# KelestZ/Latent2im

Measured on AMD Instinct MI355X. Metric: edited images/sec, higher is better.
Workload: dtype f32; 1 GPU; StyleGAN2 FFHQ-shaped 1024^2 generator (random-init, noise weights ~ 0.05: per-layer noise drawn every pass), ResNet-50 regressor, 1 CelebA attr (train.py flow), full loss (reg+content+GAN), batch 8 per GPU, linear W+ walk, eager launches; resolution=1024, global_batch=8, per_gpu_batch=8, losses=reg+content+gan, parallelism=dp1, loss_branch_streams=3, hip_graph=False

## Files before the change

include/l2i.h:

```cpp
#ifndef L2I_H
#define L2I_H

#include <stdint.h>

#ifdef __cplusplus
extern "C" {
#endif

#define L2I_OK 0
#define L2I_E_ARG (-1)
#define L2I_E_LAUNCH (-2)
#define L2I_E_UNSUPPORTED (-3)

#define L2I_ACT_NONE 0
#define L2I_ACT_LRELU 1
#define L2I_ACT_RELU 2

typedef struct l2i_conv_params {
    const float* x;
    const float* w;
    float* y;
    int32_t B, Cin, H, W, Cout, CoutP;
    int32_t KH, KW, stride, pad_y, pad_x;
    int32_t OH, OW, OHf, OWf;
// ... 19 lines not shown
    const float* res_sub;
    float res_coef;
    const float* res_coef_dev;
    const float* sq_ref;
    float* sq_out;
    int64_t w_bstride;
    int32_t out_f32;
    int32_t in_h8;
    const float* rgb_w;
    const float* rgb_bias;
    float* rgb_out;
    float* pool_out;
    uint8_t* pool_idx;
    uint8_t* mask_out;
    int32_t mask_bits;
} l2i_conv_params;
#define L2I_SQ_SLOTS 1024

int l2i_conv2d_f32(const l2i_conv_params* p, void* stream);

#define L2I_FAMILY_IMPLICIT_GEMM 0
#define L2I_FAMILY_GEMM1X1 1
#define L2I_FAMILY_CIN3 2
#define L2I_FAMILY_DIRECT_SMALL 3
int l2i_conv2d_family(const l2i_conv_params* p);

int l2i_conv_transpose2d_f32(const l2i_conv_params* p, void* stream);

int l2i_conv2d_bf16x3_f32(const l2i_conv_params* p, void* stream);

int l2i_conv_transpose2d_bf16x3_f32(const l2i_conv_params* p, void* stream);

int l2i_conv2d_wino_f32(const l2i_conv_params* p, void* stream);

int l2i_conv2d_wino4_f32(const l2i_conv_params* p, void* stream);
#define L2I_WINO4S_LEAN_CLASSES 8
int l2i_wino4s_epilogue_class(const l2i_conv_params* p);

int l2i_conv2d_h8(const l2i_conv_params* p, void* stream);
int l2i_conv_transpose2d_h8(const l2i_conv_params* p, void* stream);
// ... 169 lines not shown
```

latent2im_amd/_lib.py:

```python
import ctypes
import os

import torch

_HERE = os.path.dirname(os.path.abspath(__file__))
LIB_PATH = os.environ.get('L2I_LIB') or os.path.join(_HERE, 'libl2i_hip.so')

ACT_NONE, ACT_LRELU, ACT_RELU = 0, 1, 2

c_f = ctypes.c_float
c_i = ctypes.c_int32
c_p = ctypes.c_void_p
c_l = ctypes.c_int64


class ConvParams(ctypes.Structure):
    _fields_ = [
        ('x', c_p), ('w', c_p), ('y', c_p),
        ('B', c_i), ('Cin', c_i), ('H', c_i), ('W', c_i), ('Cout', c_i), ('CoutP', c_i),
        ('KH', c_i), ('KW', c_i), ('stride', c_i), ('pad_y', c_i), ('pad_x', c_i),
        ('OH', c_i), ('OW', c_i), ('OHf', c_i), ('OWf', c_i),
        ('oy_step', c_i), ('ox_step', c_i), ('oy_off', c_i), ('ox_off', c_i),
        ('in_scale', c_p), ('in_mask', c_p), ('mask_pos', c_f), ('mask_neg', c_f),
        ('out_scale', c_p), ('noise', c_p), ('noise_w', c_f), ('bias', c_p),
        ('residual', c_p), ('res_mask', c_p), ('out_mask', c_p),
        ('act', c_i), ('act_slope', c_f), ('act_gain', c_f), ('out_gain', c_f),
        ('accumulate', c_i), ('tile_hint', c_i),
        ('w_hi', c_p), ('w_lo', c_p),
        ('ws', c_p), ('ksplit', c_i), ('res_sub', c_p), ('res_coef', c_f), ('res_coef_dev', c_p),
        ('sq_ref', c_p), ('sq_out', c_p),
        ('w_bstride', c_l), ('out_f32', c_i),
        ('in_h8', c_i), ('rgb_w', c_p), ('rgb_bias', c_p), ('rgb_out', c_p), ('pool_out', c_p), ('pool_idx', c_p),
        ('mask_out', c_p), ('mask_bits', c_i),
    ]


SQ_SLOTS = 1024
WINO4S_LEAN_CLASSES = 8


class SegmvPart(ctypes.Structure):
    _fields_ = [('K', c_i), ('in_off_c', c_i), ('in_off_b', c_i), ('in_bstride', c_i), ('w_pitch', c_i), ('pre', c_i), ('aux_off', c_i), ('pad_', c_i),
                ('w_off', c_l)]


class SegmvSeg(ctypes.Structure):
    _fields_ = [('rows', c_i), ('nparts', c_i), ('out_off_c', c_i), ('out_off_b', c_i), ('out_bstride', c_i), ('epi', c_i), ('bias_off', c_i),
                ('e_off_c', c_i), ('e_off_b', c_i), ('e_bstride', c_i), ('rgb_off_b', c_i), ('rgb_w_off', c_i), ('part', SegmvPart * 2)]


_SIGNATURES = {
    'l2i_conv2d_f32': (c_i, [ctypes.POINTER(ConvParams), c_p]),
    'l2i_conv2d_family': (c_i, [ctypes.POINTER(ConvParams)]),
    'l2i_conv_transpose2d_f32': (c_i, [ctypes.POINTER(ConvParams), c_p]),
    'l2i_conv2d_bf16x3_f32': (c_i, [ctypes.POINTER(ConvParams), c_p]),
    'l2i_conv_transpose2d_bf16x3_f32': (c_i, [ctypes.POINTER(ConvParams), c_p]),
    'l2i_conv2d_wino_f32': (c_i, [ctypes.POINTER(ConvParams), c_p]),
    'l2i_conv2d_wino4_f32': (c_i, [ctypes.POINTER(ConvParams), c_p]),
    'l2i_wino4s_epilogue_class': (c_i, [ctypes.POINTER(ConvParams)]),
    'l2i_conv1x1_pair_f32': (c_i, [ctypes.POINTER(ConvParams), ctypes.POINTER(ConvParams), c_p]),
    'l2i_conv2d_h8': (c_i, [ctypes.POINTER(ConvParams), c_p]),
    'l2i_conv_transpose2d_h8': (c_i, [ctypes.POINTER(ConvParams), c_p]),
    'l2i_conv_img_h8': (c_i, [ctypes.POINTER(ConvParams), c_p]),
    'l2i_conv1x1_pair_h8': (c_i, [ctypes.POINTER(ConvParams), ctypes.POINTER(ConvParams), c_i, c_p]),
    'l2i_conv_chain3_h8': (c_i, [ctypes.POINTER(ConvParams), ctypes.POINTER(ConvParams), ctypes.POINTER(ConvParams), c_i, c_p]),
    'l2i_fused_bias_act_f32': (c_i, [c_p, c_p, c_p, c_p, c_l, c_l, c_l, c_i, c_i, c_f, c_f, c_p]),
    'l2i_fused_bias_act_f16': (c_i, [c_p, c_p, c_p, c_p, c_l, c_l, c_l, c_i, c_i, c_f, c_f, c_p]),
    'l2i_upfirdn2d_f16': (c_i, [c_p, c_p, c_p, c_l, c_i, c_i, c_i, c_i, c_i, c_i, c_i, c_i, c_i, c_i, c_i, c_i, c_p]),
# ... 154 lines not shown
```

latent2im_amd/conv.py:

```python

import numpy as np
import torch

from . import _lib
from ._lib import ACT_LRELU, ACT_NONE, ACT_RELU, ConvParams


import os as _os

PRECISION = _os.environ.get('L2I_PRECISION', 'f32')
H8_PRECISIONS = ('bf16', 'f16')


def h8_dtype():
    return torch.float16 if PRECISION == 'f16' else torch.bfloat16

USE_WINOGRAD = True
WINO4_MODES = ('all', 'tall', 'r4', 'off')
WINO4 = 'all'
WINO4_R4_MIN_W = 64
SPLIT_K = True
_WS = {}
USE_FUSED_TRANSPOSED = True
PROFILE = None
FAMILIES = ('implicit_gemm_f32', 'gemm1x1_f32', 'cin3_f32', 'direct_small_valu')
FAMILY_INFO = {
    'winograd_f32': ('conv_wino_kernel', 16.0 / 36.0, 157.3),
    'winograd4_f32': ('conv_wino4s_kernel', 36.0 / 144.0, 157.3),
    'implicit_gemm_f32': ('conv_mfma_kernel / conv3x3s2_dma_kernel', 1.0, 157.3),
    'gemm1x1_f32': ('gemm1x1_kernel', 1.0, 157.3),
    'transposed_f32': ('convt_mfma_kernel', 1.0, 157.3),
    'cin3_f32': ('conv_cin3_kernel', 28.0 / 27.0, 157.3),
    'direct_small_valu': ('conv_direct_small_kernel', 1.0, 157.3),
    'implicit_gemm_bf16x3': ('conv_bf16x3_pipe_kernel', 3.0, 2500.0),
    'transposed_bf16x3': ('conv_bf16x3_pipe_kernel<TR>', 3.0, 2500.0),
    'conv_h8': ('conv_h8_kernel', 1.0, 2500.0),
# ... 290 lines not shown
        B, cg, H, W, _ = x.shape
        cin = cg * 8
        assert x.dtype in (torch.bfloat16, torch.float16) and x.is_contiguous()
    else:
        B, cin, H, W = x.shape
    assert cin == F.cin and y.shape[0] == B and y.shape[1] == F.cout and y.dtype == torch.float32
    OHf, OWf = y.shape[2], y.shape[3]
    p = _conv_params(x, F.w, y, B, cin, H, W, F.cout, F.k, F.k, 2, F.pad, F.pad, (OHf + 1) // 2, (OWf + 1) // 2, OHf, OWf, 2, in_mask=in_mask, mask=mask,
                     out_gain=out_gain)
    p.in_h8 = 0 if not h8 else (2 if x.dtype == torch.float16 else 1)
    _launch('l2i_conv_transpose2d_f32', (p,), None, _transposed_meta, p, 'direct_small_valu')
    return y


def _split_k(p, px, cin, y):
    if not (SPLIT_K and px <= 2048 and cin >= 256):
        return
    ks = 16 if px <= 128 else (8 if px <= 512 else 4)
    while ks > 1 and (cin % ks or (cin // ks) % 2 or cin // ks < 16):
        ks //= 2
    if ks > 1:
        need = ks * y.numel()
        key = (y.device, torch.cuda.current_stream(y.device).cuda_stream)
        ws = _WS.get(key)
        if ws is None or ws.numel() < need:
            ws = _WS[key] = torch.empty(max(need, 1 << 22), device=y.device, dtype=torch.float32)
        p.ws, p.ksplit = _lib.fptr(ws), ks


def run_fused_transposed(F, x, y, in_scale=None, in_mask=None, mask=(1.0, 0.0), out_scale=None, out_gain=1.0, tile_hint=0):
    B, cin, H, W = x.shape
    assert cin == F.cin and y.shape[0] == B and y.shape[1] == F.cout
    OHf, OWf = y.shape[2], y.shape[3]
    p = _conv_params(x, F.w, y, B, cin, H, W, F.cout, F.k, F.k, 2, F.pad, F.pad, (OHf + 1) // 2, (OWf + 1) // 2, OHf, OWf, 2, in_scale=in_scale,
                     in_mask=in_mask, mask=mask, out_scale=out_scale, out_gain=out_gain)
    p.tile_hint = tile_hint
    name, family = 'l2i_conv_transpose2d_f32', 'transposed_f32'
    nat_h, nat_w = (H - 1) * 2 - 2 * F.pad + F.k, (W - 1) * 2 - 2 * F.pad + F.k
    if (PRECISION == 'bf16x3' and tile_hint == 0 and F.w_src is not None and W % 4 == 0 and W >= 32 and x.data_ptr() % 16 == 0
            and (in_mask is None or in_mask.data_ptr() % 16 == 0) and 0 <= OHf - nat_h <= 8 and 0 <= OWf - nat_w <= 8):
        planes = F.bf16x3_planes()
        p.w_hi, p.w_lo = _lib.ptr(planes[0]), _lib.ptr(planes[1])
# ... 356 lines not shown
```

latent2im_amd/csrc/l2i_conv.hip:

```cpp

#include <hip/hip_runtime.h>
#include <stdint.h>
#include <type_traits>
#include "l2i.h"
#include "l2i_internal.h"
#include "l2i_device.h"
#include "l2i_epilogue.h"


struct ConvLaunch {
    int tw_log2, th_log2, tb_log2;
    int tiles_x, tiles_y, bgroups, mblocks;
    int CK;
    int IH, IW, IWp;
    int planeS, plane;
    int rows_c;
    unsigned magic_iw, magic_rc, magic_ih;
    int in_elems;
    int w_vec;
    int vec_epi;
    int lstride, gstep;
    int total;
    int ksplit, cin_per;
};

template <int BM> struct WSlots { static constexpr int value = (BM == 128) ? 10 : (BM == 64 ? 8 : 4); };

template <int WM, int WN, bool VEC, bool MASK, int KT = 0>
__global__ __launch_bounds__(256, (WM * WN <= 4) ? 3 : ((WM == 2 && WN == 4) ? 2 : 1)) void conv_mfma_kernel(const l2i_conv_params p, const ConvLaunch L) {
    constexpr int BM = WM * 32;
    constexpr int NIN = VEC ? (MASK ? 4 : 8) : 12;
    constexpr int NWV = WSlots<BM>::value;
    extern __shared__ __attribute__((aligned(16))) float smem[];
    float* lds_in = smem;
    float* lds_w = smem + L.CK * L.plane;

    const int tid = threadIdx.x;
    const int lane = tid & 63;
    const int wave = tid >> 6;
    const int half = lane >> 5;
    const int j = lane & 31;
    const int KK = KT ? KT * KT : p.KH * p.KW;
    const int TW = 1 << L.tw_log2, TH = 1 << L.th_log2;
// ... 173 lines not shown
                        for (int n = 0; n < WN; ++n) bb[n] = ir[pixoff[n] + toff] * sv[n];
#pragma unroll
                        for (int m = 0; m < WM; ++m)
#pragma unroll
                            for (int n = 0; n < WN; ++n)
                                acc[m][n] = __builtin_amdgcn_mfma_f32_32x32x2f32(a[m], bb[n], acc[m][n], 0, 0, 0);
                        wr += BM;
                    }
                }
            }
        }
        __syncthreads();
    }

    const size_t plane_o = (size_t)p.OHf * p.OWf;
    if (L.ksplit > 1) {
        float* wsp = p.ws + (size_t)split * p.B * p.Cout * plane_o;
#pragma unroll
        for (int n = 0; n < WN; ++n) {
            const int pi = (wave * WN + n) * 32 + j;
            const int ox = ox0 + (pi & (TW - 1));
            const int oy = oy0 + ((pi >> L.tw_log2) & (TH - 1));
            const int bb = b0 + (pi >> (L.tw_log2 + L.th_log2));
            if (oy < p.OH && ox < p.OW && bb < p.B) {
                const size_t poff = (size_t)(oy * p.oy_step + p.oy_off) * p.OWf + ox * p.ox_step + p.ox_off;
#pragma unroll
                for (int m = 0; m < WM; ++m)
#pragma unroll
                    for (int r = 0; r < 16; ++r) {
                        const int co = m0 + 4 * half + m * 32 + (r & 3) + 8 * (r >> 2);
                        if (co < p.Cout) wsp[((size_t)bb * p.Cout + co) * plane_o + poff] = acc[m][n][r];
// ... 382 lines not shown
template <int WM, int WN>
static hipError_t launch_cfg(const l2i_conv_params& p, const ConvLaunch& L, int grid, size_t lds, bool vec, hipStream_t st) {
    const bool mask = p.in_mask != nullptr;
    if constexpr (WM == 2 && WN == 2) {
        if (!vec && p.KH == p.KW && (p.KH == 3 || p.KH == 1)) {
            hipError_t (*fn)(const l2i_conv_params&, const ConvLaunch&, int, size_t, hipStream_t) = nullptr;
            if (p.KH == 3) fn = mask ? &launch_one_kt<2, 2, true, 3> : &launch_one_kt<2, 2, false, 3>;
            else fn = mask ? &launch_one_kt<2, 2, true, 1> : &launch_one_kt<2, 2, false, 1>;
            return fn(p, L, grid, lds, st);
        }
    }
    if (vec) return mask ? launch_one<WM, WN, true, true>(p, L, grid, lds, st) : launch_one<WM, WN, true, false>(p, L, grid, lds, st);
    return mask ? launch_one<WM, WN, false, true>(p, L, grid, lds, st) : launch_one<WM, WN, false, false>(p, L, grid, lds, st);
}

static bool plan_tile(const l2i_conv_params& p, int wm, int wn, ConvLaunch& L, bool& vec, size_t& lds, long& grid) {
    const int BM = wm * 32, BN = 128 * wn;
    const int nwv = (BM == 128) ? 10 : (BM == 64 ? 8 : 4);
    L.tw_log2 = ilog2_ceil(p.OW < 32 ? p.OW : 32);
    const int TW = 1 << L.tw_log2;
    int th = BN / TW;
    const int oh_p2 = 1 << ilog2_ceil(p.OH);
    if (th > oh_p2) th = oh_p2;
    L.th_log2 = ilog2_ceil(th);
    const int TH = 1 << L.th_log2;
    L.tb_log2 = ilog2_ceil(BN / (TH * TW));
    const int TB = 1 << L.tb_log2;
    if ((size_t)TB * p.Cin * p.H * p.W * sizeof(float) >= 0xFFFFFFF0ull) return false;
    L.tiles_x = (p.OW + TW - 1) / TW;
    L.tiles_y = (p.OH + TH - 1) / TH;
    L.bgroups = (p.B + TB - 1) / TB;
// ... 12 lines not shown
    const int KK = p.KH * p.KW;
    const size_t per_c = (size_t)(L.plane + KK * BM) * sizeof(float);
    int ck = (int)((48 * 1024) / per_c);
    const int in_per_c = vec ? (L.rows_c * (L.IW / 4)) : (L.rows_c * L.IW);
    const int ck_in = ((vec ? (p.in_mask ? 4 : 8) : 12) * 256) / in_per_c;
    const int ck_w = (nwv * 256) / (KK * BM / 4);
    if (ck > ck_in) ck = ck_in;
    if (ck > ck_w) ck = ck_w;
    if (p.in_scale && ck > (256 >> L.tb_log2)) ck = 256 >> L.tb_log2;
    ck &= ~1;
    if (ck < 2) return false;
    const int cin_even = (p.Cin + 1) & ~1;
    if (ck > cin_even) ck = cin_even;
    L.ksplit = 1;
    L.cin_per = p.Cin;
    if (p.ksplit > 1 && p.ws) {
        const int per = p.Cin / p.ksplit;
        if (per >= 2 && per * p.ksplit == p.Cin && (per % 2) == 0) {
            while (ck > 2 && (per % ck) != 0) ck -= 2;
            if ((per % ck) == 0) { L.ksplit = p.ksplit; L.cin_per = per; }
        }
    }
    L.CK = ck;
    L.in_elems = ck * in_per_c;
    L.w_vec = ck * KK * BM / 4;
    L.magic_iw = magic_for((unsigned)L.IW);
    L.magic_rc = magic_for((unsigned)L.rows_c);
    L.magic_ih = magic_for((unsigned)L.IH);
    lds = per_c * ck + (size_t)(ck << L.tb_log2) * sizeof(float);
    L.vec_epi = (l2i_epilogue_vec_ok(p) && L.tw_log2 >= 2) ? 1 : 0;
    if (L.vec_epi && lds < 4 * 32 * 64 * sizeof(float)) lds = 4 * 32 * 64 * sizeof(float);
    grid = (long)L.bgroups * L.tiles_y * L.tiles_x * L.mblocks * L.ksplit;
    if (!(lds <= 64 * 1024 && grid > 0 && grid <= 0x7ffffff0L)) return false;
    L.total = (int)grid;
    grid = (grid + 7) & ~7L;
    return true;
}

extern "C" int l2i_conv2d_family(const l2i_conv_params* pp) {
    if (!pp) return L2I_E_ARG;
    const l2i_conv_params& p = *pp;
    if (p.Cout <= 4 && p.stride == 1 && p.KH <= 16 && p.tile_hint == 0 && !p.out_scale && !p.noise && !p.bias && !p.residual && !p.out_mask &&
        p.act == L2I_ACT_NONE)
        return L2I_FAMILY_DIRECT_SMALL;
    if (p.tile_hint == 0 && l2i_gemm1x1_eligible(p)) return L2I_FAMILY_GEMM1X1;
    if (p.tile_hint == 0 && l2i_cin3_eligible(p)) return L2I_FAMILY_CIN3;
    return L2I_FAMILY_IMPLICIT_GEMM;
}

extern "C" int l2i_conv2d_f32(const l2i_conv_params* pp, void* stream) {
    if (!pp) return l2i_set_error(L2I_E_ARG, "conv2d: null params");
// ... 10 lines not shown
    if (p.res_sub && !p.residual) return l2i_set_error(L2I_E_ARG, "conv2d: res_sub needs residual");
    if ((p.sq_ref || p.sq_out) && !(p.sq_ref && p.sq_out && (((uintptr_t)p.sq_ref) % 16) == 0 && p.tile_hint == 0 && l2i_cin3_eligible(p)))
        return l2i_set_error(L2I_E_UNSUPPORTED, "conv2d: sq_ref / sq_out are fused in l2i_conv2d_wino_f32 and in the <= 3-input-channel kernel only");
    if (p.oy_step <= 0 || p.ox_step <= 0 || (p.OH - 1) * p.oy_step + p.oy_off >= p.OHf || (p.OW - 1) * p.ox_step + p.ox_off >= p.OWf ||
        p.oy_off < 0 || p.ox_off < 0)
        return l2i_set_error(L2I_E_ARG, "conv2d: output window exceeds the output tensor");
    if ((((uintptr_t)p.w) % 16) != 0) return l2i_set_error(L2I_E_ARG, "conv2d: packed weights must be 16-byte aligned");
    if ((size_t)p.Cin * p.H * p.W * sizeof(float) >= 0xFFFFFFF0ull || (size_t)p.Cin * p.KH * p.KW * p.CoutP * sizeof(float) >= 0xFFFFFFF0ull)
        return l2i_set_error(L2I_E_UNSUPPORTED, "conv2d: one sample / the weight pack must stay below 4 GiB (32-bit buffer offsets)");

    const int family = l2i_conv2d_family(pp);
    if (family == L2I_FAMILY_DIRECT_SMALL) return launch_direct_small(p, (hipStream_t)stream);
    if (family == L2I_FAMILY_GEMM1X1) return l2i_launch_gemm1x1(p, (hipStream_t)stream);
    if (family == L2I_FAMILY_CIN3) return l2i_launch_cin3(p, (hipStream_t)stream);
    if (p.tile_hint == 0 && l2i_conv3x3s2_eligible(p)) return l2i_launch_conv3x3s2(p, (hipStream_t)stream);

    ConvLaunch L, Lbest;
    bool vec = false, vbest = false;
    size_t lds = 0, lbest = 0;
    long grid = 0, gbest = -1;
    int sel = -1;
    if (p.tile_hint > 0) {
        if (p.tile_hint > kNumTiles) return l2i_set_error(L2I_E_ARG, "conv2d: tile_hint out of range");
        sel = p.tile_hint - 1;
        if (!plan_tile(p, kTiles[sel].wm, kTiles[sel].wn, Lbest, vbest, lbest, gbest))
            return l2i_set_error(L2I_E_UNSUPPORTED, "conv2d: requested tile cannot be staged for this problem");
    } else {
        static const int kCand[6] = {1, 2, 3, 4, 0, 0};
        static const int kOcc[6] = {3, 3, 3, 4, 1, 1};
        static const double kEff[6] = {1.0, 1.0, 1.04, 1.08, 1.0, 1.0};
// ... 38 lines not shown
```

latent2im_amd/csrc/l2i_convt.hip:

```cpp

#include <hip/hip_runtime.h>
#include <stdint.h>
#include "l2i.h"
#include "l2i_internal.h"
#include "l2i_device.h"


struct ConvTLaunch {
    int TW, TH, tb_log2;
    unsigned magic_tw, magic_th;
    int ksplit, cin_per;
    int tiles_x, tiles_y, bgroups, mblocks;
    int CK, IH, IW, IWp, planeS, plane, rows_c;
    unsigned magic_iw, magic_rc, magic_ih;
    int in_elems, w_vec;
    int total;
    int nslots;
};


template <int K, int PAD> struct TrGeom {
    static constexpr int k0(int pi) { return (pi + PAD) % 2; }
    static constexpr int A(int pi) { return (K - k0(pi) + 1) / 2; }
    static constexpr int d(int pi) { return (pi + PAD - k0(pi)) / 2; }
    static constexpr int pad(int pi) { return A(pi) - 1 - d(pi); }
    static constexpr int P = pad(0) > pad(1) ? pad(0) : pad(1);
    static constexpr int q_(int pi) { return A(pi) - 1 - pad(pi); }
    static constexpr int Q = q_(0) > q_(1) ? q_(0) : q_(1);
};

template <int K, int PAD, int WN, bool MASK, bool DMAIN = false>
__global__ __launch_bounds__(256, WN == 1 ? 3 : 2) void convt_mfma_kernel(const l2i_conv_params p, const ConvTLaunch L) {
    using G = TrGeom<K, PAD>;
    constexpr int BM = 32, KK = K * K, NIN = DMAIN ? 1 : 12, P = G::P, Q = G::Q;
    static_assert(!(DMAIN && MASK), "the DMA path has no VALU pass for a gradient mask");
    extern __shared__ __attribute__((aligned(16))) float smem[];
    const int stage_f = L.CK * L.plane + L.CK * KK * BM + ((L.CK << L.tb_log2) + 3 & ~3);

    const int tid = threadIdx.x, lane = tid & 63, wave = tid >> 6, half = lane >> 5, j = lane & 31;
    const int TW = L.TW, TH = L.TH;
    int bid = (int)((blockIdx.x & 7) * (gridDim.x >> 3) + (blockIdx.x >> 3));
    if (bid >= L.total) return;
    const int mblk = bid % L.mblocks; bid /= L.mblocks;
    const int tx = bid % L.tiles_x; bid /= L.tiles_x;
    const int ty = bid % L.tiles_y; bid /= L.tiles_y;
    const int bgrp = bid % L.bgroups;
// ... 254 lines not shown
                    }
                }
            }
        }
        if constexpr (DMAIN) {
            asm volatile("s_waitcnt vmcnt(0)" ::: "memory");
            if (c0 + L.CK < c_end) store_sc(st ^ 1);
        } else {
            if (more) asm volatile("s_waitcnt vmcnt(%0)" :: "n"(NREG) : "memory");
            else asm volatile("s_waitcnt vmcnt(0)" ::: "memory");
        }
        __syncthreads();
    }

    const size_t plane_o = (size_t)p.OHf * p.OWf;
    if (L.ksplit > 1) {
        float* wsp = p.ws + (size_t)split * p.B * p.Cout * plane_o;
#pragma unroll
        for (int n = 0; n < WN; ++n) {
            const int pi = (wave * WN + n) * 32 + j;
            const int rowi = (int)fast_div((unsigned)pi, L.magic_tw);
            const int tbi = (int)fast_div((unsigned)rowi, L.magic_th);
            const int tcol = tx0 + (pi - rowi * TW), trow = ty0 + (rowi - tbi * TH);
            const int bb = tbi < (1 << L.tb_log2) ? b0 + tbi : p.B;
            if (bb < p.B) {
#pragma unroll
                for (int q = 0; q < 4; ++q) {
                    const int oy = 2 * trow + (q >> 1), ox = 2 * tcol + (q & 1);
                    if (oy < p.OHf && ox < p.OWf) {
#pragma unroll
                        for (int r = 0; r < 16; ++r) {
// ... 46 lines not shown
                    } else {
                        dst[0] = v.x;
                        if (ox + 1 < p.OWf) dst[1] = v.y;
                        if (ox + 2 < p.OWf) dst[2] = v.z;
                    }
                }
            }
        }
    }
}

static int ilog2c(int v) { int l = 0; while ((1 << l) < v) ++l; return l; }
static unsigned magic_of(unsigned d) { return (unsigned)((0x100000000ULL + d - 1) / d); }

template <int K, int PAD, int WN>
static int launch_convt(const l2i_conv_params& p, hipStream_t st) {
    using G = TrGeom<K, PAD>;
    constexpr int BM = 32, BN = 128 * WN, KK = K * K;
    ConvTLaunch L;
    const int Ty = (p.OHf + 1) / 2, Tx = (p.OWf + 1) / 2;
    int TW, TH;
    if (Tx < 32) {
        TW = 1 << ilog2c(Tx);
        int th = BN / TW;
        const int ty_p2 = 1 << ilog2c(Ty);
        if (th > ty_p2) th = ty_p2;
        TH = 1 << ilog2c(th);
        L.tb_log2 = ilog2c(BN / (TH * TW));
    } else {
        long best = -1;
        TW = 32; TH = BN / 32;
// ... 9 lines not shown
    L.magic_tw = TW == 1 ? 0u : magic_of((unsigned)TW);
    L.magic_th = TH == 1 ? 0u : magic_of((unsigned)TH);
    const int TB = 1 << L.tb_log2;
    if ((size_t)TB * p.Cin * p.H * p.W * sizeof(float) >= 0xFFFFFFF0ull) return l2i_set_error(L2I_E_UNSUPPORTED, "conv_transpose2d: sample group >= 4 GiB");
    L.tiles_x = (Tx + TW - 1) / TW;
    L.tiles_y = (Ty + TH - 1) / TH;
    L.bgroups = (p.B + TB - 1) / TB;
    L.mblocks = (p.CoutP + BM - 1) / BM;
    L.IH = TH + G::P + G::Q;
    L.IW = TW + G::P + G::Q;
    L.IWp = L.IW | 1;
    L.planeS = L.IH * L.IWp;
    L.plane = (TB * L.planeS + 3) & ~3;
    L.rows_c = TB * L.IH;
    L.nslots = 0;
    const bool dma_in = K == 3 && !p.in_mask && TB == 1 && Tx >= 32 && !(p.ksplit > 1 && p.ws) && L.IH * L.IW <= 6 * 64 &&
                        (size_t)p.Cin * p.H * p.W * sizeof(float) < 0x7FFF0000ull;
    if (dma_in) {
        L.IWp = L.IW;
        L.planeS = L.IH * L.IW;
        L.nslots = (L.planeS + 63) / 64;
        L.plane = 6 * 64 + 32;
    }
    const size_t per_c = (size_t)(L.plane + KK * BM) * sizeof(float);
    int ck = (int)(((dma_in && WN == 1 ? 24 : 36) * 1024) / per_c);
    const int ck_in = dma_in ? 16 : (12 * 256) / (L.rows_c * L.IW);
    if (ck > ck_in) ck = ck_in;
    if (p.in_scale && ck > (256 >> L.tb_log2)) ck = 256 >> L.tb_log2;
    constexpr int CKQ = (K == 3) ? 4 : 2;
    if ((p.Cin % CKQ) != 0) return l2i_set_error(L2I_E_UNSUPPORTED, K == 3 ? "conv_transpose2d: Cin must be a multiple of 4" : "conv_transpose2d: Cin must be even");
    ck &= ~(CKQ - 1);
    if (ck > p.Cin) ck = p.Cin;
    while (ck > CKQ && (p.Cin % ck) != 0) ck -= CKQ;
    if (ck < CKQ) return l2i_set_error(L2I_E_UNSUPPORTED, "conv_transpose2d: tile cannot be staged");
    L.ksplit = 1;
    L.cin_per = p.Cin;
    if (p.ksplit > 1 && p.ws) {
        const int per = p.Cin / p.ksplit;
        if (per >= CKQ && per * p.ksplit == p.Cin && (per % CKQ) == 0) {
            while (ck > CKQ && (per % ck) != 0) ck -= CKQ;
            if ((per % ck) == 0) { L.ksplit = p.ksplit; L.cin_per = per; }
        }
    }
    if (dma_in) {
        int plane = 6 * 64;
        while (((ck / 2) * plane) % 64 != 32 && plane < 6 * 64 + 64) ++plane;
        if (((ck / 2) * plane) % 64 != 32) plane = 6 * 64 + 16;
        L.plane = plane;
    }
    L.CK = ck;
    L.in_elems = ck * L.rows_c * L.IW;
    L.w_vec = ck * KK * BM / 4;
    L.magic_iw = magic_of((unsigned)L.IW);
    L.magic_rc = magic_of((unsigned)L.rows_c);
    L.magic_ih = magic_of((unsigned)L.IH);
    size_t lds = 2 * ((size_t)(L.plane + KK * BM) * sizeof(float) * ck + (size_t)(((ck << L.tb_log2) + 3) & ~3) * sizeof(float));
    if (lds < 4 * 32 * 64 * sizeof(float)) lds = 4 * 32 * 64 * sizeof(float);
    long grid = (long)L.bgroups * L.tiles_y * L.tiles_x * L.mblocks * L.ksplit;
    if (grid <= 0 || grid > 0x7ffffff0L) return l2i_set_error(L2I_E_ARG, "conv_transpose2d: grid too large");
    L.total = (int)grid;
    grid = (grid + 7) & ~7L;
    if (lds > (dma_in ? 80 : 64) * 1024) return l2i_set_error(L2I_E_UNSUPPORTED, "conv_transpose2d: tile cannot be staged");
    if constexpr (K == 3) {
        if (dma_in) L2I_ONCE_PER_DEVICE((void)hipFuncSetAttribute(reinterpret_cast<const void*>(&convt_mfma_kernel<K, PAD, WN, false, true>),
                                                                  hipFuncAttributeMaxDynamicSharedMemorySize, 80 * 1024));
    }
    if (p.in_mask) hipLaunchKernelGGL((convt_mfma_kernel<K, PAD, WN, true>), dim3((unsigned)grid), dim3(256), lds, st, p, L);
    else if constexpr (K == 3) {
        if (dma_in) hipLaunchKernelGGL((convt_mfma_kernel<K, PAD, WN, false, true>), dim3((unsigned)grid), dim3(256), lds, st, p, L);
        else hipLaunchKernelGGL((convt_mfma_kernel<K, PAD, WN, false>), dim3((unsigned)grid), dim3(256), lds, st, p, L);
    } else hipLaunchKernelGGL((convt_mfma_kernel<K, PAD, WN, false>), dim3((unsigned)grid), dim3(256), lds, st, p, L);
    L2I_CHECK_LAUNCH();
    if (L.ksplit > 1) {
        l2i_conv_params q = p;
        q.ksplit = L.ksplit;
        q.OH = p.OHf; q.OW = p.OWf; q.oy_step = q.ox_step = 1; q.oy_off = q.ox_off = 0;
        return l2i_launch_splitk_epilogue(q, st);
    }
    return L2I_OK;
}

extern "C" int l2i_conv_transpose2d_f32(const l2i_conv_params* pp, void* stream) {
    if (!pp) return l2i_set_error(L2I_E_ARG, "conv_transpose2d: null params");
    const l2i_conv_params& p = *pp;
    if (!p.x || !p.w || !p.y) return l2i_set_error(L2I_E_ARG, "conv_transpose2d: null tensor");
    if (const char* m = l2i_unsupported_v5_fields(p, false, false, true)) return l2i_set_error(L2I_E_UNSUPPORTED, m);
    if (p.B <= 0 || p.Cin <= 0 || p.Cout <= 0 || p.H <= 0 || p.W <= 0) return l2i_set_error(L2I_E_ARG, "conv_transpose2d: non-positive dimension");
    if (p.KH != p.KW || p.pad_y != p.pad_x) return l2i_set_error(L2I_E_ARG, "conv_transpose2d: square kernels / symmetric padding only");
    if (p.sq_ref || p.sq_out) return l2i_set_error(L2I_E_UNSUPPORTED, "conv_transpose2d: sq_ref / sq_out are fused in l2i_conv2d_wino_f32 only");
    if (p.CoutP == 4 && p.Cout <= 3) {
        if (p.bias || p.noise || p.residual || p.res_mask || p.res_sub || p.out_mask || p.act != L2I_ACT_NONE)
            return l2i_set_error(L2I_E_UNSUPPORTED, "conv_transpose2d: only in_mask / out_gain / accumulate are fused in the small-output kernel");
        if (!l2i_convt_small_eligible(p)) return l2i_set_error(L2I_E_UNSUPPORTED, "conv_transpose2d(small): 7x7 / pad 3, W % 4 == 0, OWf % 4 == 0, aligned tensors, no scales");
        if (p.OHf > 2 * p.H + 8 || p.OWf > 2 * p.W + 8) return l2i_set_error(L2I_E_ARG, "conv_transpose2d(small): output window too large for the input");
        return l2i_launch_convt_small(p, (hipStream_t)stream);
    }
    if (p.in_h8) return l2i_set_error(L2I_E_UNSUPPORTED, "conv_transpose2d: in_h8 is built for the 7x7 / pad 3 kernel onto <= 3 channels only");
    if (p.CoutP < p.Cout || (p.CoutP % 32) != 0) return l2i_set_error(L2I_E_ARG, "conv_transpose2d: CoutP must be Cout rounded up to 32");
    const int full_h = (p.H - 1) * 2 - 2 * p.pad_y + p.KH, full_w = (p.W - 1) * 2 - 2 * p.pad_x + p.KW;
    if (p.OHf < full_h || p.OWf < full_w || p.OHf > full_h + 8 || p.OWf > full_w + 8)
        return l2i_set_error(L2I_E_ARG, "conv_transpose2d: output must be the natural size (or up to 8 larger: zero rows / columns)");
    if (p.bias || p.noise || p.residual || p.res_mask || p.res_sub || p.out_mask || p.act != L2I_ACT_NONE || p.accumulate)
        return l2i_set_error(L2I_E_UNSUPPORTED, "conv_transpose2d: only in_scale / in_mask / out_scale / out_gain are fused here");
    if ((((uintptr_t)p.w) % 16) != 0) return l2i_set_error(L2I_E_ARG, "conv_transpose2d: packed weights must be 16-byte aligned");
    if ((size_t)p.Cin * p.KH * p.KW * p.CoutP * sizeof(float) >= 0xFFFFFFF0ull) return l2i_set_error(L2I_E_UNSUPPORTED, "conv_transpose2d: weight pack >= 4 GiB");
    hipStream_t st = (hipStream_t)stream;
    const bool narrow = p.tile_hint == 1 || (p.tile_hint != 2 && ((p.OWf + 1) / 2 <= 33 || p.W <= 33));
    if (p.KH == 3 && p.pad_y == 0) return narrow ? launch_convt<3, 0, 1>(p, st) : launch_convt<3, 0, 2>(p, st);
    if (p.KH == 3 && p.pad_y == 1) return narrow ? launch_convt<3, 1, 1>(p, st) : launch_convt<3, 1, 2>(p, st);
    if (p.KH == 7 && p.pad_y == 3) return launch_convt<7, 3, 2>(p, st);
    return l2i_set_error(L2I_E_UNSUPPORTED, "conv_transpose2d: fused kernel built for (K,pad) in {(3,0),(3,1),(7,3)}");
}
```

latent2im_amd/csrc/l2i_internal.h:

```cpp
#ifndef L2I_INTERNAL_H
#define L2I_INTERNAL_H
#include <hip/hip_runtime.h>
#include <atomic>
#include <cstdint>

int l2i_set_error(int code, const char* msg);

struct l2i_conv_params;
bool l2i_gemm1x1_eligible(const l2i_conv_params& p);
int l2i_launch_gemm1x1(const l2i_conv_params& p, hipStream_t st);
bool l2i_cin3_eligible(const l2i_conv_params& p);
int l2i_launch_cin3(const l2i_conv_params& p, hipStream_t st);
bool l2i_convt_small_eligible(const l2i_conv_params& p);
int l2i_launch_convt_small(const l2i_conv_params& p, hipStream_t st);
bool l2i_conv3x3s2_eligible(const l2i_conv_params& p);
int l2i_launch_conv3x3s2(const l2i_conv_params& p, hipStream_t st);
int l2i_launch_splitk_epilogue(const l2i_conv_params& q, hipStream_t st);

static inline const char* l2i_unsupported_v5_fields(const l2i_conv_params& p, bool allow_rgb, bool allow_pool, bool allow_in_h8) {
    if (!allow_rgb && (p.rgb_w || p.rgb_bias || p.rgb_out)) return "rgb_w / rgb_bias / rgb_out are fused in l2i_conv2d_h8 only";
    if (!allow_pool && (p.pool_out || p.pool_idx)) return "pool_out / pool_idx are fused in l2i_conv2d_wino4_f32 only";
    if (!allow_in_h8 && p.in_h8) return "in_h8 is read by the 7x7 kernel of l2i_conv_transpose2d_f32 only";
    if (!allow_rgb && (p.mask_out || p.mask_bits)) return "mask_out / mask_bits (one-bit activation masks) belong to l2i_conv2d_h8 / l2i_conv_transpose2d_h8";
    return nullptr;
}

#define L2I_CHECK_LAUNCH()                                                      \
    do {                                                                        \
        hipError_t e_ = hipGetLastError();                                      \
        if (e_ != hipSuccess) return l2i_set_error(L2I_E_LAUNCH, hipGetErrorString(e_)); \
    } while (0)

// ... 20 lines not shown
```

Baseline: 82.50 images/s.

## Add in-kernel split-K reduction with atomic counters for small-map convolutions

Adds a small-map split-K path for 3x3 convolutions and 3x3 transposed convolutions with few output positions. Each split writes its tile partials to a per-tile slab, and the last-arriving block, found through an atomic counter, sums them in place and runs the epilogue. This replaces the separate split-K epilogue launch and picks the range count from a target block count, aiming for more parallelism on small maps with fewer launches. It needs a persistent counter buffer that must reset correctly, a larger workspace, and more workspace traffic.

Measured after the change: 82.46 images/s. No clear change (-0.1%).

```diff
diff --git a/include/l2i.h b/include/l2i.h
--- a/include/l2i.h
+++ b/include/l2i.h
@@ -57,6 +57,10 @@
     uint8_t* pool_idx;
     uint8_t* mask_out;
     int32_t mask_bits;
+    uint32_t* sk_count;
+    int64_t ws_cap;
+    int32_t sk_count_n;
+    int32_t sk_ranges;
 } l2i_conv_params;
 #define L2I_SQ_SLOTS 1024
 
@@ -67,6 +71,8 @@
 #define L2I_FAMILY_CIN3 2
 #define L2I_FAMILY_DIRECT_SMALL 3
 int l2i_conv2d_family(const l2i_conv_params* p);
+
+int l2i_smallmap_plan(const l2i_conv_params* p, int transposed, int64_t* out);
 
 int l2i_conv_transpose2d_f32(const l2i_conv_params* p, void* stream);
 
diff --git a/latent2im_amd/_lib.py b/latent2im_amd/_lib.py
--- a/latent2im_amd/_lib.py
+++ b/latent2im_amd/_lib.py
@@ -32,6 +32,7 @@
         ('w_bstride', c_l), ('out_f32', c_i),
         ('in_h8', c_i), ('rgb_w', c_p), ('rgb_bias', c_p), ('rgb_out', c_p), ('pool_out', c_p), ('pool_idx', c_p),
         ('mask_out', c_p), ('mask_bits', c_i),
+        ('sk_count', c_p), ('ws_cap', c_l), ('sk_count_n', c_i), ('sk_ranges', c_i),
     ]
 
 
@@ -52,6 +53,7 @@
 _SIGNATURES = {
     'l2i_conv2d_f32': (c_i, [ctypes.POINTER(ConvParams), c_p]),
     'l2i_conv2d_family': (c_i, [ctypes.POINTER(ConvParams)]),
+    'l2i_smallmap_plan': (c_i, [ctypes.POINTER(ConvParams), c_i, ctypes.POINTER(c_l)]),
     'l2i_conv_transpose2d_f32': (c_i, [ctypes.POINTER(ConvParams), c_p]),
     'l2i_conv2d_bf16x3_f32': (c_i, [ctypes.POINTER(ConvParams), c_p]),
     'l2i_conv_transpose2d_bf16x3_f32': (c_i, [ctypes.POINTER(ConvParams), c_p]),
diff --git a/latent2im_amd/conv.py b/latent2im_amd/conv.py
--- a/latent2im_amd/conv.py
+++ b/latent2im_amd/conv.py
@@ -20,6 +20,11 @@
 WINO4 = 'all'
 WINO4_R4_MIN_W = 64
 SPLIT_K = True
+SMALLMAP = True
+SMALLMAP_WS = 1 << 24
+SMALLMAP_COUNTERS = 4096
+SMALLMAP_RANGES = 0
+SPLIT_K_MIN_CIN = 256
 _WS = {}
 USE_FUSED_TRANSPOSED = True
 PROFILE = None
@@ -340,7 +345,7 @@
 
 
 def _split_k(p, px, cin, y):
-    if not (SPLIT_K and px <= 2048 and cin >= 256):
+    if not (SPLIT_K and px <= 2048 and cin >= SPLIT_K_MIN_CIN):
         return
     ks = 16 if px <= 128 else (8 if px <= 512 else 4)
     while ks > 1 and (cin % ks or (cin // ks) % 2 or cin // ks < 16):
@@ -348,10 +353,14 @@
     if ks > 1:
         need = ks * y.numel()
         key = (y.device, torch.cuda.current_stream(y.device).cuda_stream)
-        ws = _WS.get(key)
+        ws, cnt = _WS.get(key, (None, None))
         if ws is None or ws.numel() < need:
-            ws = _WS[key] = torch.empty(max(need, 1 << 22), device=y.device, dtype=torch.float32)
+            ws = torch.empty(max(need, SMALLMAP_WS), device=y.device, dtype=torch.float32)
+            cnt = cnt if cnt is not None else torch.zeros(SMALLMAP_COUNTERS, device=y.device, dtype=torch.int32)
+            _WS[key] = (ws, cnt)
         p.ws, p.ksplit = _lib.fptr(ws), ks
+        if SMALLMAP:
+            p.sk_count, p.ws_cap, p.sk_count_n, p.sk_ranges = _lib.ptr(cnt), ws.numel(), cnt.numel(), SMALLMAP_RANGES
 
 
 def run_fused_transposed(F, x, y, in_scale=None, in_mask=None, mask=(1.0, 0.0), out_scale=None, out_gain=1.0, tile_hint=0):
diff --git a/latent2im_amd/csrc/l2i_conv.hip b/latent2im_amd/csrc/l2i_conv.hip
--- a/latent2im_amd/csrc/l2i_conv.hip
+++ b/latent2im_amd/csrc/l2i_conv.hip
@@ -6,6 +6,7 @@
 #include "l2i_internal.h"
 #include "l2i_device.h"
 #include "l2i_epilogue.h"
+#include "l2i_smallmap.h"
 
 
 struct ConvLaunch {
@@ -26,7 +27,7 @@
 
 template <int BM> struct WSlots { static constexpr int value = (BM == 128) ? 10 : (BM == 64 ? 8 : 4); };
 
-template <int WM, int WN, bool VEC, bool MASK, int KT = 0>
+template <int WM, int WN, bool VEC, bool MASK, int KT = 0, bool SK = false>
 __global__ __launch_bounds__(256, (WM * WN <= 4) ? 3 : ((WM == 2 && WN == 4) ? 2 : 1)) void conv_mfma_kernel(const l2i_conv_params p, const ConvLaunch L) {
     constexpr int BM = WM * 32;
     constexpr int NIN = VEC ? (MASK ? 4 : 8) : 12;
@@ -230,7 +231,16 @@
     }
 
     const size_t plane_o = (size_t)p.OHf * p.OWf;
-    if (L.ksplit > 1) {
+    if constexpr (SK) {
+        if (L.ksplit > 1) {
+            constexpr int TF = WM * WN * 16 * 256;
+            const int tile = ((bgrp * L.tiles_y + ty) * L.tiles_x + tx) * L.mblocks + mblk;
+            float* slabs = p.ws + (size_t)tile * L.ksplit * TF;
+            l2i_sk_store<WM * WN>(slabs + (size_t)split * TF, &acc[0][0]);
+            if (!l2i_sk_arrive(p.sk_count + tile, L.ksplit, smem)) return;
+            l2i_sk_sum<WM * WN>(slabs, L.ksplit, &acc[0][0]);
+        }
+    } else if (L.ksplit > 1) {
         float* wsp = p.ws + (size_t)split * p.B * p.Cout * plane_o;
 #pragma unroll
         for (int n = 0; n < WN; ++n) {
@@ -643,7 +653,7 @@
     return mask ? launch_one<WM, WN, false, true>(p, L, grid, lds, st) : launch_one<WM, WN, false, false>(p, L, grid, lds, st);
 }
 
-static bool plan_tile(const l2i_conv_params& p, int wm, int wn, ConvLaunch& L, bool& vec, size_t& lds, long& grid) {
+static bool plan_tile(const l2i_conv_params& p, int wm, int wn, ConvLaunch& L, bool& vec, size_t& lds, long& grid, bool sk = false) {
     const int BM = wm * 32, BN = 128 * wn;
     const int nwv = (BM == 128) ? 10 : (BM == 64 ? 8 : 4);
     L.tw_log2 = ilog2_ceil(p.OW < 32 ? p.OW : 32);
@@ -686,7 +696,14 @@
     if (ck > cin_even) ck = cin_even;
     L.ksplit = 1;
     L.cin_per = p.Cin;
-    if (p.ksplit > 1 && p.ws) {
+    if (sk) {
+        while (ck > 2 && (p.Cin % ck) != 0) ck -= 2;
+        if ((p.Cin % ck) != 0) return false;
+        const long long tiles = (long long)L.bgroups * L.tiles_y * L.tiles_x * L.mblocks;
+        const l2i_sk_plan pl = l2i_sk_choose_ranges(p.Cin, ck, tiles, (long long)BM * BN, p.ws_cap, p.sk_count_n, p.sk_ranges > 0 ? p.sk_ranges : 0);
+        L.ksplit = pl.ranges;
+        L.cin_per = pl.cin_per;
+    } else if (p.ksplit > 1 && p.ws) {
         const int per = p.Cin / p.ksplit;
         if (per >= 2 && per * p.ksplit == p.Cin && (per % 2) == 0) {
             while (ck > 2 && (per % ck) != 0) ck -= 2;
@@ -707,6 +724,45 @@
     L.total = (int)grid;
     grid = (grid + 7) & ~7L;
     return true;
+}
+
+static bool smallmap_conv_takes(const l2i_conv_params& p) {
+    if (p.sk_ranges == 0 && !(p.stride == 2 && (long long)p.B * p.OH * p.OW > 1024)) return false;
+    return p.sk_count && p.ws && p.ws_cap > 0 && p.sk_count_n > 0 && p.tile_hint == 0 && p.KH == 3 && p.KW == 3 && p.pad_y == p.pad_x &&
+           ((p.stride == 1 && p.pad_y == 1) || (p.stride == 2 && (p.pad_y == 0 || p.pad_y == 1))) && (p.Cin % 2) == 0 && p.Cin >= 16 && p.Cout > 4 &&
+           (p.CoutP % 32) == 0 && !p.sq_ref && (long long)p.B * p.OH * p.OW <= L2I_SK_MAX_POSITIONS;
+}
+
+static int plan_smallmap_conv(const l2i_conv_params& p, ConvLaunch& L, size_t& lds, long& grid) {
+    const long long px = (long long)p.B * p.OH * p.OW;
+    int sel = px <= 128 ? 4 : (px <= 1024 ? 3 : 1);
+    if (kTiles[sel].wm * 32 > p.CoutP) sel = 4;
+    bool vec = false;
+    if (!plan_tile(p, kTiles[sel].wm, kTiles[sel].wn, L, vec, lds, grid, true) || vec) return -1;
+    return sel;
+}
+
+template <int WM, int WN>
+static hipError_t launch_smallmap_conv(const l2i_conv_params& p, const ConvLaunch& L, int grid, size_t lds, hipStream_t st) {
+    if (p.in_mask) hipLaunchKernelGGL((conv_mfma_kernel<WM, WN, false, true, 3, true>), dim3(grid), dim3(256), lds, st, p, L);
+    else hipLaunchKernelGGL((conv_mfma_kernel<WM, WN, false, false, 3, true>), dim3(grid), dim3(256), lds, st, p, L);
+    return hipGetLastError();
+}
+
+extern "C" int l2i_smallmap_plan(const l2i_conv_params* pp, int transposed, int64_t* out) {
+    if (!pp || !out) return 0;
+    if (transposed) return l2i_convt_smallmap_plan(*pp, out);
+    const l2i_conv_params& p = *pp;
+    if (l2i_conv2d_family(pp) != L2I_FAMILY_IMPLICIT_GEMM || !smallmap_conv_takes(p)) return 0;
+    ConvLaunch L;
+    size_t lds = 0;
+    long grid = 0;
+    const int sel = plan_smallmap_conv(p, L, lds, grid);
+    if (sel < 0) return 0;
+    const long long tiles = L.total / L.ksplit;
+    out[0] = L.ksplit; out[1] = L.cin_per; out[2] = L.CK; out[3] = tiles; out[4] = L.total;
+    out[5] = L.ksplit > 1 ? (long long)L.ksplit * tiles * kTiles[sel].wm * kTiles[sel].wn * 4096 : 0;
+    return 1;
 }
 
 extern "C" int l2i_conv2d_family(const l2i_conv_params* pp) {
@@ -747,6 +803,21 @@
     if (family == L2I_FAMILY_GEMM1X1) return l2i_launch_gemm1x1(p, (hipStream_t)stream);
     if (family == L2I_FAMILY_CIN3) return l2i_launch_cin3(p, (hipStream_t)stream);
     if (p.tile_hint == 0 && l2i_conv3x3s2_eligible(p)) return l2i_launch_conv3x3s2(p, (hipStream_t)stream);
+
+    if (smallmap_conv_takes(p)) {
+        ConvLaunch Ls;
+        size_t lds_s = 0;
+        long grid_s = 0;
+        const int s = plan_smallmap_conv(p, Ls, lds_s, grid_s);
+        if (s >= 0) {
+            hipError_t es;
+            if (s == 1) es = launch_smallmap_conv<2, 2>(p, Ls, (int)grid_s, lds_s, (hipStream_t)stream);
+            else if (s == 3) es = launch_smallmap_conv<2, 1>(p, Ls, (int)grid_s, lds_s, (hipStream_t)stream);
+            else es = launch_smallmap_conv<1, 1>(p, Ls, (int)grid_s, lds_s, (hipStream_t)stream);
+            if (es != hipSuccess) return l2i_set_error(L2I_E_LAUNCH, hipGetErrorString(es));
+            return L2I_OK;
+        }
+    }
 
     ConvLaunch L, Lbest;
     bool vec = false, vbest = false;
diff --git a/latent2im_amd/csrc/l2i_convt.hip b/latent2im_amd/csrc/l2i_convt.hip
--- a/latent2im_amd/csrc/l2i_convt.hip
+++ b/latent2im_amd/csrc/l2i_convt.hip
@@ -4,6 +4,7 @@
 #include "l2i.h"
 #include "l2i_internal.h"
 #include "l2i_device.h"
+#include "l2i_smallmap.h"
 
 
 struct ConvTLaunch {
@@ -29,7 +30,7 @@
     static constexpr int Q = q_(0) > q_(1) ? q_(0) : q_(1);
 };
 
-template <int K, int PAD, int WN, bool MASK, bool DMAIN = false>
+template <int K, int PAD, int WN, bool MASK, bool DMAIN = false, bool SK = false>
 __global__ __launch_bounds__(256, WN == 1 ? 3 : 2) void convt_mfma_kernel(const l2i_conv_params p, const ConvTLaunch L) {
     using G = TrGeom<K, PAD>;
     constexpr int BM = 32, KK = K * K, NIN = DMAIN ? 1 : 12, P = G::P, Q = G::Q;
@@ -314,7 +315,16 @@
     }
 
     const size_t plane_o = (size_t)p.OHf * p.OWf;
-    if (L.ksplit > 1) {
+    if constexpr (SK) {
+        if (L.ksplit > 1) {
+            constexpr int TF = 4 * WN * 16 * 256;
+            const int tile = ((bgrp * L.tiles_y + ty) * L.tiles_x + tx) * L.mblocks + mblk;
+            float* slabs = p.ws + (size_t)tile * L.ksplit * TF;
+            l2i_sk_store<4 * WN>(slabs + (size_t)split * TF, &acc[0][0]);
+            if (!l2i_sk_arrive(p.sk_count + tile, L.ksplit, smem)) return;
+            l2i_sk_sum<4 * WN>(slabs, L.ksplit, &acc[0][0]);
+        }
+    } else if (L.ksplit > 1) {
         float* wsp = p.ws + (size_t)split * p.B * p.Cout * plane_o;
 #pragma unroll
         for (int n = 0; n < WN; ++n) {
@@ -391,7 +401,7 @@
 static unsigned magic_of(unsigned d) { return (unsigned)((0x100000000ULL + d - 1) / d); }
 
 template <int K, int PAD, int WN>
-static int launch_convt(const l2i_conv_params& p, hipStream_t st) {
+static int launch_convt(const l2i_conv_params& p, hipStream_t st, bool sk = false, int64_t* plan_out = nullptr) {
     using G = TrGeom<K, PAD>;
     constexpr int BM = 32, BN = 128 * WN, KK = K * K;
     ConvTLaunch L;
@@ -431,7 +441,7 @@
     L.plane = (TB * L.planeS + 3) & ~3;
     L.rows_c = TB * L.IH;
     L.nslots = 0;
-    const bool dma_in = K == 3 && !p.in_mask && TB == 1 && Tx >= 32 && !(p.ksplit > 1 && p.ws) && L.IH * L.IW <= 6 * 64 &&
+    const bool dma_in = K == 3 && !p.in_mask && TB == 1 && Tx >= 32 && !(p.ksplit > 1 && p.ws) && !sk && L.IH * L.IW <= 6 * 64 &&
                         (size_t)p.Cin * p.H * p.W * sizeof(float) < 0x7FFF0000ull;
     if (dma_in) {
         L.IWp = L.IW;
@@ -452,7 +462,12 @@
     if (ck < CKQ) return l2i_set_error(L2I_E_UNSUPPORTED, "conv_transpose2d: tile cannot be staged");
     L.ksplit = 1;
     L.cin_per = p.Cin;
-    if (p.ksplit > 1 && p.ws) {
+    if (sk) {
+        const long long tiles = (long long)L.bgroups * L.tiles_y * L.tiles_x * L.mblocks;
+        const l2i_sk_plan pl = l2i_sk_choose_ranges(p.Cin, ck, tiles, (long long)4 * BM * BN, p.ws_cap, p.sk_count_n, p.sk_ranges > 0 ? p.sk_ranges : 0);
+        L.ksplit = pl.ranges;
+        L.cin_per = pl.cin_per;
+    } else if (p.ksplit > 1 && p.ws) {
         const int per = p.Cin / p.ksplit;
         if (per >= CKQ && per * p.ksplit == p.Cin && (per % CKQ) == 0) {
             while (ck > CKQ && (per % ck) != 0) ck -= CKQ;
@@ -478,6 +493,20 @@
     L.total = (int)grid;
     grid = (grid + 7) & ~7L;
     if (lds > (dma_in ? 80 : 64) * 1024) return l2i_set_error(L2I_E_UNSUPPORTED, "conv_transpose2d: tile cannot be staged");
+    if (plan_out) {
+        const long long tiles = L.total / L.ksplit;
+        plan_out[0] = L.ksplit; plan_out[1] = L.cin_per; plan_out[2] = L.CK; plan_out[3] = tiles; plan_out[4] = L.total;
+        plan_out[5] = L.ksplit > 1 ? (long long)L.ksplit * tiles * 4 * BM * BN : 0;
+        return L2I_OK;
+    }
+    if constexpr (K == 3 && WN == 1) {
+        if (sk) {
+            if (p.in_mask) hipLaunchKernelGGL((convt_mfma_kernel<K, PAD, WN, true, false, true>), dim3((unsigned)grid), dim3(256), lds, st, p, L);
+            else hipLaunchKernelGGL((convt_mfma_kernel<K, PAD, WN, false, false, true>), dim3((unsigned)grid), dim3(256), lds, st, p, L);
+            L2I_CHECK_LAUNCH();
+            return L2I_OK;
+        }
+    }
     if constexpr (K == 3) {
         if (dma_in) L2I_ONCE_PER_DEVICE((void)hipFuncSetAttribute(reinterpret_cast<const void*>(&convt_mfma_kernel<K, PAD, WN, false, true>),
                                                                   hipFuncAttributeMaxDynamicSharedMemorySize, 80 * 1024));
@@ -495,6 +524,19 @@
         return l2i_launch_splitk_epilogue(q, st);
     }
     return L2I_OK;
+}
+
+static bool smallmap_convt_takes(const l2i_conv_params& p) {
+    if (p.sk_ranges == 0 && !((long long)p.B * p.H * p.W > 128 && (long long)p.B * p.H * p.W <= 1024)) return false;
+    return p.sk_count && p.ws && p.ws_cap > 0 && p.sk_count_n > 0 && p.tile_hint == 0 && p.KH == 3 && p.KW == 3 && p.pad_y == p.pad_x &&
+           (p.pad_y == 0 || p.pad_y == 1) && (p.Cin % 4) == 0 && p.Cin >= 16 && ((p.OWf + 1) / 2 <= 33 || p.W <= 33) &&
+           (long long)p.B * p.H * p.W <= L2I_SK_MAX_POSITIONS;
+}
+
+int l2i_convt_smallmap_plan(const l2i_conv_params& p, int64_t* out) {
+    if (!p.x || !p.w || !p.y || p.CoutP == 4 || (p.CoutP % 32) != 0 || !smallmap_convt_takes(p)) return 0;
+    const int rc = p.pad_y == 0 ? launch_convt<3, 0, 1>(p, nullptr, true, out) : launch_convt<3, 1, 1>(p, nullptr, true, out);
+    return rc == L2I_OK ? 1 : 0;
 }
 
 extern "C" int l2i_conv_transpose2d_f32(const l2i_conv_params* pp, void* stream) {
@@ -523,6 +565,7 @@
     if ((size_t)p.Cin * p.KH * p.KW * p.CoutP * sizeof(float) >= 0xFFFFFFF0ull) return l2i_set_error(L2I_E_UNSUPPORTED, "conv_transpose2d: weight pack >= 4 GiB");
     hipStream_t st = (hipStream_t)stream;
     const bool narrow = p.tile_hint == 1 || (p.tile_hint != 2 && ((p.OWf + 1) / 2 <= 33 || p.W <= 33));
+    if (smallmap_convt_takes(p)) return p.pad_y == 0 ? launch_convt<3, 0, 1>(p, st, true) : launch_convt<3, 1, 1>(p, st, true);
     if (p.KH == 3 && p.pad_y == 0) return narrow ? launch_convt<3, 0, 1>(p, st) : launch_convt<3, 0, 2>(p, st);
     if (p.KH == 3 && p.pad_y == 1) return narrow ? launch_convt<3, 1, 1>(p, st) : launch_convt<3, 1, 2>(p, st);
     if (p.KH == 7 && p.pad_y == 3) return launch_convt<7, 3, 2>(p, st);
diff --git a/latent2im_amd/csrc/l2i_internal.h b/latent2im_amd/csrc/l2i_internal.h
--- a/latent2im_amd/csrc/l2i_internal.h
+++ b/latent2im_amd/csrc/l2i_internal.h
@@ -16,6 +16,7 @@
 bool l2i_conv3x3s2_eligible(const l2i_conv_params& p);
 int l2i_launch_conv3x3s2(const l2i_conv_params& p, hipStream_t st);
 int l2i_launch_splitk_epilogue(const l2i_conv_params& q, hipStream_t st);
+int l2i_convt_smallmap_plan(const l2i_conv_params& p, int64_t* out);
 
 static inline const char* l2i_unsupported_v5_fields(const l2i_conv_params& p, bool allow_rgb, bool allow_pool, bool allow_in_h8) {
     if (!allow_rgb && (p.rgb_w || p.rgb_bias || p.rgb_out)) return "rgb_w / rgb_bias / rgb_out are fused in l2i_conv2d_h8 only";
diff --git a/latent2im_amd/csrc/l2i_smallmap.h b/latent2im_amd/csrc/l2i_smallmap.h
--- /dev/null
+++ b/latent2im_amd/csrc/l2i_smallmap.h
@@ -0,0 +1,108 @@
+#ifndef L2I_SMALLMAP_H
+#define L2I_SMALLMAP_H
+
+#define L2I_SK_MAX_POSITIONS 2048
+#define L2I_SK_MAX_RANGES 32
+#define L2I_SK_TARGET_BLOCKS 512
+
+struct l2i_sk_plan {
+    int ranges;
+    int cin_per;
+    long long ws_floats;
+};
+
+static inline l2i_sk_plan l2i_sk_choose_ranges(int cin, int chunk, long long tiles, long long tile_floats, long long ws_cap, long long counters, int forced) {
+    l2i_sk_plan r = {1, cin, 0};
+    if (chunk <= 0 || cin <= 0 || (cin % chunk) != 0 || tiles <= 0 || tile_floats <= 0 || tiles > counters) return r;
+    const long long nchunks = cin / chunk;
+    long long cap = ws_cap / (tiles * tile_floats);
+    if (cap > L2I_SK_MAX_RANGES) cap = L2I_SK_MAX_RANGES;
+    if (cap > nchunks) cap = nchunks;
+    if (cap < 2) return r;
+    long long per;
+    if (forced > 0) {
+        const long long want = forced < cap ? forced : cap;
+        per = (nchunks + want - 1) / want;
+    } else {
+        long long want = (L2I_SK_TARGET_BLOCKS + tiles - 1) / tiles;
+        if (want > cap) want = cap;
+        per = nchunks / want;
+        while ((nchunks + per - 1) / per > cap) ++per;
+    }
+    const long long ranges = (nchunks + per - 1) / per;
+    if (ranges < 2) return r;
+    r.ranges = (int)ranges;
+    r.cin_per = (int)(per * chunk);
+    r.ws_floats = ranges * tiles * tile_floats;
+    return r;
+}
+
+#ifdef __HIPCC__
+#include <hip/hip_runtime.h>
+#include "l2i_device.h"
+
+template <int NACC>
+__device__ __forceinline__ void l2i_sk_store(float* slab, const f32x16* acc) {
+    float4* dst = reinterpret_cast<float4*>(slab) + threadIdx.x;
+#pragma unroll
+    for (int a = 0; a < NACC; ++a)
+#pragma unroll
+        for (int q = 0; q < 4; ++q) dst[(a * 4 + q) * 256] = make_float4(acc[a][4 * q], acc[a][4 * q + 1], acc[a][4 * q + 2], acc[a][4 * q + 3]);
+}
+
+template <int NACC>
+__device__ __forceinline__ void l2i_sk_sum(const float* slabs, int ranges, f32x16* acc) {
+#pragma unroll
+    for (int a = 0; a < NACC; ++a)
+#pragma unroll
+        for (int r = 0; r < 16; ++r) acc[a][r] = 0.f;
+    constexpr int SB = NACC == 1 ? 8 : (NACC == 2 ? 4 : 1);
+    constexpr int SLAB4 = NACC * 4 * 256;
+    const float4* src = reinterpret_cast<const float4*>(slabs) + threadIdx.x;
+    int s = 0;
+    for (; s + SB <= ranges; s += SB) {
+        float4 v[SB][NACC * 4];
+#pragma unroll
+        for (int u = 0; u < SB; ++u)
+#pragma unroll
+            for (int k = 0; k < NACC * 4; ++k) v[u][k] = src[(size_t)(s + u) * SLAB4 + k * 256];
+#pragma unroll
+        for (int u = 0; u < SB; ++u)
+#pragma unroll
+            for (int k = 0; k < NACC * 4; ++k) {
+                acc[k >> 2][4 * (k & 3)] += v[u][k].x; acc[k >> 2][4 * (k & 3) + 1] += v[u][k].y;
+                acc[k >> 2][4 * (k & 3) + 2] += v[u][k].z; acc[k >> 2][4 * (k & 3) + 3] += v[u][k].w;
+            }
+    }
+    for (; s < ranges; ++s) {
+#pragma unroll
+        for (int k = 0; k < NACC * 4; ++k) {
+            const float4 v = src[(size_t)s * SLAB4 + k * 256];
+            acc[k >> 2][4 * (k & 3)] += v.x; acc[k >> 2][4 * (k & 3) + 1] += v.y; acc[k >> 2][4 * (k & 3) + 2] += v.z; acc[k >> 2][4 * (k & 3) + 3] += v.w;
+        }
+    }
+}
+
+__device__ __forceinline__ bool l2i_sk_arrive(unsigned* cnt, int ranges, float* lds) {
+    asm volatile("s_waitcnt vmcnt(0)" ::: "memory");
+    __syncthreads();
+    volatile unsigned* flag = reinterpret_cast<volatile unsigned*>(lds);
+    if (threadIdx.x == 0) {
+        __builtin_amdgcn_fence(__ATOMIC_RELEASE, "agent");
+        asm volatile("s_waitcnt vmcnt(0)" ::: "memory");
+        const unsigned prev = __hip_atomic_fetch_add(cnt, 1u, __ATOMIC_RELAXED, __HIP_MEMORY_SCOPE_AGENT);
+        const bool last = prev == (unsigned)(ranges - 1);
+        if (last) {
+            __hip_atomic_store(cnt, 0u, __ATOMIC_RELAXED, __HIP_MEMORY_SCOPE_AGENT);
+            __builtin_amdgcn_fence(__ATOMIC_ACQUIRE, "agent");
+            asm volatile("s_waitcnt vmcnt(0)" ::: "memory");
+        }
+        *flag = last ? 1u : 0u;
+    }
+    __syncthreads();
+    const bool last = *flag != 0u;
+    __syncthreads();
+    return last;
+}
+#endif
+#endif
```
